# rlvc/FEALESS

Hardware: AMD Instinct MI355X
Metric: frames/sec (640x480 RGB-D x N templates, 20 ICP iters) (higher is better)
Workload: dtype u8

## Files before the change

### fealess_amd/csrc/fl_context.hip

```cpp
#include "fl_internal.h"
#include <stdlib.h>
#include <stdarg.h>
#include <string.h>
#include <algorithm>

int fl_set_error(fl_context *ctx, int code, const char *fmt, ...)
{
  if (ctx) {
    va_list ap;
    va_start(ap, fmt);
    vsnprintf(ctx->err, sizeof(ctx->err), fmt, ap);
    va_end(ap);
  }
  return code;
}

int fl_scratch(fl_context *ctx, size_t bytes, void **out)
{
  if (int rc = fl_context_join(ctx)) return rc;
  if (bytes > ctx->scratch_bytes) {
    if (ctx->scratch) {
      FL_HIP(ctx, hipStreamSynchronize(ctx->stream));
      FL_HIP(ctx, hipFree(ctx->scratch));
      ctx->scratch = nullptr;
// ... 38 lines not shown
  FL_HIP(ctx, hipStreamSynchronize(ctx->stream));
  if (ctx->icp_stream) FL_HIP(ctx, hipStreamSynchronize(ctx->icp_stream));
  ctx->icp_pending = false;
  return FL_OK;
}

int fl_icp_stream(fl_context *ctx, hipStream_t *out)
{
  const long mode = ctx->opt.pipeline_icp;
  if (ctx->icp_stream && ctx->icp_stream_mode != mode) {
    FL_HIP(ctx, hipStreamSynchronize(ctx->icp_stream));
    FL_HIP(ctx, hipStreamDestroy(ctx->icp_stream));
    ctx->icp_stream = nullptr;
  }
  if (!ctx->icp_stream) {
    int least = 0, greatest = 0;
    FL_HIP(ctx, hipDeviceGetStreamPriorityRange(&least, &greatest));
    FL_HIP(ctx, hipStreamCreateWithPriority(&ctx->icp_stream, hipStreamNonBlocking, mode == 2 ? greatest : (mode == 3 ? least : 0)));
    ctx->icp_stream_mode = mode;
  }
  if (!ctx->ev_icp_tail) FL_HIP(ctx, hipEventCreateWithFlags(&ctx->ev_icp_tail, hipEventDisableTiming));
  *out = ctx->icp_stream;
  return FL_OK;
}

extern "C" int fl_abi_version(void) { return FL_ABI_VERSION; }

struct FlOptionName { const char *name, *env; long fl_context::Options::*field; bool hex; long lo, hi; };
static const FlOptionName fl_option_names[] = {
  {"scan_prune", "FL_SCAN_PRUNE", &fl_context::Options::scan_prune, false, 0, 1},
  {"scan_prune_mid", "FL_SCAN_PRUNE_MID", &fl_context::Options::scan_prune_mid, true, -1, 0xFF},
  {"scan_prune_lanes", "FL_SCAN_PRUNE_LANES", &fl_context::Options::scan_prune_lanes, false, 0, 1},
  {"scan_prune_step", "FL_SCAN_PRUNE_STEP", &fl_context::Options::scan_prune_step, false, 0, 8},
  {"icp_wide", "FL_ICP_WIDE", &fl_context::Options::icp_wide, false, -1, 1},
  {"icp_occ", "FL_ICP_OCC", &fl_context::Options::icp_occ, false, 0, 5},
  {"icp_order", "FL_ICP_ORDER", &fl_context::Options::icp_order, false, 0, 1},
  {"icp_wg_per_cu", "FL_ICP_WG_PER_CU", &fl_context::Options::icp_wg_per_cu, false, 0, 3},
  {"eager_frontend", "FL_EAGER_FRONTEND", &fl_context::Options::eager_frontend, false, 0, 1},
  {"dev_poison", "FL_DEV_POISON", &fl_context::Options::dev_poison, false, 0, 1},
  {"ws_pad", "FL_DEV_WS_PAD", &fl_context::Options::ws_pad, false, 0, 16l << 20},
  {"pipeline_icp", "FL_PIPELINE_ICP", &fl_context::Options::pipeline_icp, false, 0, 3},
  {"frontend_chunk_rows", "FL_FRONTEND_CHUNK_ROWS", &fl_context::Options::frontend_chunk_rows, false, 0, 60 * 1024},
  {"scan_run", "FL_SCAN_RUN", &fl_context::Options::scan_run, false, 0, 64},
  {"refine_lds", "FL_REFINE_LDS", &fl_context::Options::refine_lds, false, 0, 2},
  {"refine_lds_bytes", "FL_REFINE_LDS_BYTES", &fl_context::Options::refine_lds_bytes, false, 0, FL_REFINE_LDS_BYTES},
  {"verify_fused", "FL_VERIFY_FUSED", &fl_context::Options::verify_fused, false, 0, 1},
  {"verify_fused_px", "FL_VERIFY_FUSED_PX", &fl_context::Options::verify_fused_px, false, 0, FL_VERIFY_FUSED_PX},
};

static bool fl_option_valid(const FlOptionName &o, long v)
{
  if (v < o.lo || v > o.hi) return false;
  if (o.field == &fl_context::Options::frontend_chunk_rows) return v % 60 == 0;
  if (o.field == &fl_context::Options::verify_fused_px) return v == 0 || v >= FL_WAVE;
  if (o.field == &fl_context::Options::scan_prune_step) return v == 0 || v == 2 || v == 4 || v == 8;
  return o.field != &fl_context::Options::icp_occ || v == 0 || v >= 4;
}

extern "C" int fl_context_create(int device, fl_context **out)
{
  if (!out) return FL_ERR_INVALID;
  *out = nullptr;
  int n = 0;
  if (hipGetDeviceCount(&n) != hipSuccess || n <= 0) return FL_ERR_NO_DEVICE;
  if (device < 0 || device >= n) return FL_ERR_INVALID;
  fl_context *ctx = new fl_context();
  ctx->device = device;
  if (hipSetDevice(device) != hipSuccess ||
      hipStreamCreateWithFlags(&ctx->own_stream, hipStreamNonBlocking) != hipSuccess) {
    delete ctx;
    return FL_ERR_HIP;
  }
  ctx->stream = ctx->own_stream;
  {
    hipDeviceProp_t prop;
    if (hipGetDeviceProperties(&prop, device) == hipSuccess && prop.multiProcessorCount > 0) ctx->cus = prop.multiProcessorCount;
  }
  for (const FlOptionName &o : fl_option_names)
    if (const char *e = getenv(o.env)) {
      const long v = o.hex ? (long)strtoul(e, nullptr, 16) : atol(e);
      if (fl_option_valid(o, v)) ctx->opt.*(o.field) = v;
    }
  *out = ctx;
  return FL_OK;
}

extern "C" void *fl_context_get_stream(fl_context *ctx) { return ctx ? (void *)ctx->stream : nullptr; }
extern "C" int fl_context_get_device(const fl_context *ctx) { return ctx ? ctx->device : -1; }
// ... 525 lines not shown
              ff.qx = (int16_t)((f.x - rx) / Tl);
              ff.qy = (int16_t)((f.y - ry) / Tl);
              ff.label = (uint8_t)f.label;
              ff.pad = 0;
            }
            fine_feat.push_back(ff);
            const FlRect one = {ff.x, ff.y, ff.x, ff.y};
            box = fl_rect_union(box, one);
          }
          fine_hdr.push_back(h);
          fine_box.push_back(FlFineBox{(int16_t)box.x0, (int16_t)box.y0, (int16_t)box.x1, (int16_t)box.y1});
          all = fl_rect_union(all, box);
        }
        if (all.x1 >= all.x0) {
          const FlLevelGeom &gl = det->geom[l];
          const int ww = std::min(all.x1 - all.x0 + 15 * gl.T + 1 + 3, (gl.w + 3) & ~3);
          const int hh = std::min(all.y1 - all.y0 + 15 * gl.T + 1, gl.h);
          const long bytes = (long)fl_refine_pitch(ww, fl_refine_qmask(gl.T)) * hh;
          det->refine_window_max[l] = std::max(det->refine_window_max[l], bytes);
        }
      }
    }
  }
  det->n_pyr = g_idx;
  det->scan_bytes_per_frame = scan_bytes;

  int rc;
  {
    std::vector<FlScanItem> items;
    fl_build_scan_items(scan_hdr, g_idx, M, det->geom[L - 1].WH, det->geom[L - 1].zero_off, scan_off, items);
    det->n_scan_items = (int)items.size();
    det->scan_item_g.clear();
    for (const FlScanItem &it : items) det->scan_item_g.push_back(it.g);
    if ((rc = upload(ctx, items, &det->d_scan_items))) return rc;
  }
  if ((rc = upload(ctx, scan_off, &det->d_scan_off))) return rc;
  if ((rc = upload(ctx, fine_hdr, &det->d_fine_hdr))) return rc;
  if ((rc = upload(ctx, fine_feat, &det->d_fine_feat))) return rc;
  if ((rc = upload(ctx, fine_box, &det->d_fine_box))) return rc;
  if ((rc = upload(ctx, pyr, &det->d_pyr))) return rc;
  if ((rc = upload(ctx, poses, &det->d_poses))) return rc;
  if ((rc = upload(ctx, class_first, &det->d_class_first))) return rc;
  if ((rc = fl_apply_class_filter(det))) return rc;
  {
    const uint16_t **tmp = nullptr;
    if ((rc = upload(ctx, depth_ptrs, (const uint16_t ***)&tmp))) return rc;
    det->d_depth_ptrs = tmp;
  }

  det->w0 = w0;
  det->h0 = h0;
  det->max_batch = max_batch;
  det->eager_env = ctx->opt.eager_frontend != 0;
  det->poison_env = ctx->opt.dev_poison != 0;
  if ((rc = layout_workspace(det, cap))) return rc;
  if ((rc = fl_icp_prepare(det))) return rc;
  FL_HIP(ctx, hipMalloc((void **)&det->d_results, sizeof(fl_recognition_result) * (size_t)max_batch));
  FL_HIP(ctx, hipHostMalloc((void **)&det->h_results, sizeof(fl_recognition_result) * 2 * (size_t)max_batch,
                            hipHostMallocDefault));
  for (auto &e : det->ev) FL_HIP(ctx, hipEventCreate(&e));
  for (int b = 0; b < 2; ++b) {
    FL_HIP(ctx, hipEventCreateWithFlags(&det->ev_done[b], hipEventDisableTiming));
    FL_HIP(ctx, hipEventCreateWithFlags(&det->ev_set_read[b], hipEventDisableTiming));
  }
  det->finalized = true;
  return FL_OK;
// ... 2 lines not shown
```

### fealess_amd/csrc/fl_internal.h

```cpp
#pragma once
#include <hip/hip_runtime.h>
#include <cmath>
#include <stdint.h>
#include <stdio.h>
#include <string>
#include <vector>
#include "../../include/fealess_hip.h"

#define FL_WAVE 64

struct fl_context {
  int device = 0;
  hipStream_t own_stream = nullptr;
  hipStream_t stream = nullptr;
  hipStream_t icp_stream = nullptr;
  long icp_stream_mode = 0;
  hipEvent_t ev_icp_tail = nullptr;
  bool icp_pending = false;
  char err[512] = {0};
  void *scratch = nullptr;
  size_t scratch_bytes = 0;
  void *pinned = nullptr;
  size_t pinned_bytes = 0;
  int cus = 256;
  struct Options {
    long scan_prune = 1;
    long scan_prune_mid = -1;
    long scan_prune_lanes = 1;
    long scan_prune_step = 0;
    long icp_wide = -1;
    long icp_occ = 0;
    long icp_order = 1;
    long icp_wg_per_cu = 0;
    long eager_frontend = 0;
    long dev_poison = 0;
    long ws_pad = 0;
    long pipeline_icp = 3;
    long frontend_chunk_rows = 0;
    long scan_run = 0;
    long refine_lds = 0;
    long refine_lds_bytes = 0;
    long verify_fused = 0;
    long verify_fused_px = 0;
  } opt;
  bool verify_fused_attr = false;
  int detectors = 0;
  bool destroy_pending = false;
};

int fl_set_error(fl_context *ctx, int code, const char *fmt, ...);
int fl_scratch(fl_context *ctx, size_t bytes, void **out);
int fl_pinned(fl_context *ctx, size_t bytes, void **out);
int fl_context_join(fl_context *ctx);
int fl_context_sync_all(fl_context *ctx);
int fl_icp_stream(fl_context *ctx, hipStream_t *out);

#define FL_HIP(ctx, call)                                                                  \
  do {                                                                                     \
    hipError_t e_ = (call);                                                                \
    if (e_ != hipSuccess)                                                                  \
      return fl_set_error((ctx), FL_ERR_HIP, "%s:%d: %s -> %s", __FILE__, __LINE__, #call, \
                          hipGetErrorString(e_));                                          \
// ... 141 lines not shown

struct FlClass {
  std::string id;
  int n_pyramids = 0;
  std::vector<fl_template> templates;
  std::vector<fl_feature> features;
  std::vector<float> poses;
  int first_g = 0;
  uint16_t *d_depths = nullptr;
  std::vector<uint8_t> has_depth;
  int dw = 0, dh = 0;
};

struct FlBatch {
  int n = 0;
  const uint16_t *depth = nullptr;
  size_t depth_stride = 0;
  bool match_only = false;
};

struct fl_detector {
  fl_context *ctx = nullptr;
  int M = 0, L = 0;
  int T[FL_MAX_LEVELS] = {0};
  std::vector<FlClass> classes;
  bool finalized = false;
  int w0 = 0, h0 = 0, max_batch = 0, cap = 0;
  bool cap_hard = false;
  int n_pyr = 0;
  FlLevelGeom geom[FL_MAX_LEVELS];

  FlScanItem *d_scan_items = nullptr;
  int n_scan_items = 0;
  std::vector<int32_t> scan_item_g;
  uint32_t *d_scan_off = nullptr;
  FlFineHdr *d_fine_hdr = nullptr;
  FlFineBox *d_fine_box = nullptr;
  long refine_window_max[FL_MAX_LEVELS] = {0};
  int refine_ran[FL_MAX_LEVELS] = {0};
  FlFineFeat *d_fine_feat = nullptr;
  FlPyrInfo *d_pyr = nullptr;
  int *d_class_first = nullptr;
  uint8_t *d_item_enabled = nullptr;
  std::vector<std::string> class_filter;
  float *d_poses = nullptr;
  const uint16_t **d_depth_ptrs = nullptr;
  int depth_w = 0, depth_h = 0;
  int max_tw = 0, max_th = 0;

  uint8_t *d_ws = nullptr;
  size_t ws_stride = 0;
  size_t off_bgr = 0, off_depth = 0, off_cand = 0, off_count = 0, off_keys = 0, off_match = 0;
  size_t off_icp = 0, off_tmp = 0;
  size_t off_count_set[2] = {0, 0}, off_match_set[2] = {0, 0};
  int set = 0;
  hipEvent_t ev_set_read[2] = {nullptr, nullptr};
  bool set_busy[2] = {false, false};
  size_t off_tiles = 0;
  bool lazy_capable = false;
  bool lazy = false;
  bool eager_env = false, poison_env = false;
  const uint8_t *lazy_bgr = nullptr;
  hipStream_t copy_stream = nullptr;
  uint8_t *d_in[2] = {nullptr, nullptr};
  hipEvent_t ev_up[2] = {nullptr, nullptr}, ev_read[2] = {nullptr, nullptr};
  bool read_pending[2] = {false, false};
// ... 182 lines not shown
```

### fealess_amd/csrc/fl_linemod.hip

```cpp
#include "fl_internal.h"
#include <limits.h>
#include <string.h>
#include <algorithm>
#include <type_traits>

__global__ __launch_bounds__(256) void k_build_lm_generic(FlPlanes pl, int n_mod, int w, int h, int T, int W, int WH, uint32_t stride)
{
  const int p = blockIdx.x * 256 + threadIdx.x;
  const int gi = blockIdx.y;
  const int frame = blockIdx.z / n_mod, m = blockIdx.z - frame * n_mod;
  const uint8_t *q = pl.in + (size_t)frame * pl.in_stride + pl.in_off[m];
  uint8_t *out = pl.out + (size_t)frame * pl.out_stride + pl.out_off[m];
  if (p >= WH) return;
  const int gy = gi / T, gx = gi - gy * T;
  const int yt = p / W, xt = p - yt * W;
  const int y = yt * T + gy, x = xt * T + gx;
  unsigned b = 0;
  const int rmax = min(T, h - y), cmax = min(T, w - x);
  for (int r = 0; r < rmax; ++r) {
    const uint8_t *row = q + (size_t)(y + r) * w + x;
    for (int c = 0; c < cmax; ++c) b |= row[c];
  }
  const unsigned bb = b | (b << 8);
#pragma unroll
// ... 396 lines not shown
  unsigned prune_mid;
  int prune_lanes;
  uint16_t *dbg;
  int dbg_first, dbg_count;
};

typedef unsigned int u32x4 __attribute__((ext_vector_type(4)));
typedef unsigned short u16x2 __attribute__((ext_vector_type(2)));
__device__ __forceinline__ u16x2 pk_bytes_max(uint32_t a)
{
  const uint32_t lo = a & 0x00FF00FFu, hi = (a >> 8) & 0x00FF00FFu;
  return __builtin_elementwise_max(__builtin_bit_cast(u16x2, lo), __builtin_bit_cast(u16x2, hi));
}
__device__ __forceinline__ uint4 ld16(const uint8_t *p)
{
  uint4 v;
  __builtin_memcpy(&v, p, 16);
  return v;
}
#define FL_CONST_AS __attribute__((address_space(4)))
__device__ __forceinline__ uint32_t sload1(const void *p) { return *(const FL_CONST_AS uint32_t *)(uintptr_t)p; }
__device__ __forceinline__ uint32_t rl(uint32_t v, int l) { return (uint32_t)__builtin_amdgcn_readlane((int)v, l); }

#ifndef FL_SCAN_PRUNE_MID
#define FL_SCAN_PRUNE_MID 0x7Fu
#endif
#ifndef FL_SCAN_OFFSETS_AHEAD
#define FL_SCAN_OFFSETS_AHEAD 1
#endif
#ifndef FL_SCAN_WPE
#define FL_SCAN_WPE 5
#endif
#ifndef FL_SCAN_WPE_PRUNED
#define FL_SCAN_WPE_PRUNED 6
#endif
#ifndef FL_SCAN_STEP
#define FL_SCAN_STEP 4
#endif
#ifndef FL_SCAN_TAIL_ALWAYS
#define FL_SCAN_TAIL_ALWAYS 0
#endif
#ifdef FL_SCAN_STATS
#define FL_SCAN_STATS_N (4 + 2 * FL_MAX_FEATURES + 1)
__device__ unsigned long long d_scan_stats[FL_SCAN_STATS_N];
#define FL_SCAN_STAT(i, v) do { if (lane == 0) atomicAdd(&d_scan_stats[i], (unsigned long long)(v)); } while (0)
#else
#define FL_SCAN_STAT(i, v) do { } while (0)
#endif
template <int N> struct ScanInt { static constexpr int value = N; };
template <int WPE, int STEP>
__global__ __launch_bounds__(256) __attribute__((amdgpu_waves_per_eu(WPE, WPE))) void k_scan(ScanArgs a)
{
  static_assert(STEP == 8 || STEP == 4 || STEP == 2, "a group of eight offsets is cut into equal parts");
  const int wave = threadIdx.x >> 6, lane = threadIdx.x & 63;
  const int xcd = blockIdx.x & 7, q = blockIdx.x >> 3;
  const int frame = xcd + 8 * (q / a.bpf);
  if (frame >= a.n_frames) return;
  int it = __builtin_amdgcn_readfirstlane(((q % a.bpf) * 4 + wave) * a.wave_step);
  if (it >= a.n_items) return;
  const int l7 = lane & 7;
  auto request_item = [&](int idx) {
    const uint32_t *p = lane < 16 ? (const uint32_t *)(a.items + idx) + lane : (const uint32_t *)(a.enabled + (idx & ~3));
    return *p;
  };
  uint32_t rec = request_item(it);
  const uint8_t *lm[FL_MAX_MODALITIES];
  for (int m = 0; m < FL_MAX_MODALITIES; ++m) lm[m] = a.ws + (size_t)frame * a.ws_stride + a.lm_off[m];
  const float thr100 = a.threshold / 100.f;
  const unsigned lane_off = (unsigned)lane * 16u;
  const int dbg_first = a.dbg_first;
  const unsigned dbg_count = (unsigned)a.dbg_count;
  const FL_CONST_AS ScanArgs *ka = (const FL_CONST_AS ScanArgs *)__builtin_amdgcn_kernarg_segment_ptr();

  auto scan_item = [&](const uint32_t r) {
    const int g = (int)rl(r, 8), chunk = (int)(rl(r, 9) & 0xFFFFu), nf_all = (int)(rl(r, 9) >> 16);
    const int rP[FL_MAX_MODALITIES] = {(int)rl(r, 10), (int)rl(r, 13)}, rB[FL_MAX_MODALITIES] = {(int)rl(r, 11), (int)rl(r, 14)};
    const uint32_t rN[FL_MAX_MODALITIES] = {rl(r, 12), rl(r, 15)};
    const int j0 = chunk * 1024 + lane * 16;

    uint32_t tot[16];
#pragma unroll
    for (int i = 0; i < 16; ++i) tot[i] = 0;
    const int prune_threshold = (int)(2 * nf_all + thr100 * (2 * nf_all) + 0.5f);
    const bool tapped = (unsigned)(g - dbg_first) < dbg_count;
    const bool prune = a.prune && !tapped;
    const unsigned mid = prune ? a.prune_mid : 0u;
    const bool by_lane = prune && a.prune_lanes;
    uint64_t alive = ~0ull;
    auto still = [&](bool reachable) {
      const uint64_t b = __ballot(reachable) & alive;
      alive = by_lane || b == 0ull ? b : ~0ull;
      return alive != 0ull;
    };
    [[maybe_unused]] int f_done = 0;
    FL_SCAN_STAT(0, 1);
    uint32_t ov = r;
    int o_at = (rN[0] & 0xFFFFu) ? rB[0] : -1;
    int nf = 0;
#pragma unroll
    for (int m = 0; m < FL_MAX_MODALITIES; ++m) {
      if (m >= a.M) break;
      const int P = rP[m], off_begin = rB[m], n_pad = (int)(rN[m] & 0xFFFFu), h_nf = (int)(rN[m] >> 16);
      uint32_t mx_tot = 0;
      if (prune && m > 0) {
#pragma unroll
        for (int i = 0; i < 16; ++i) mx_tot = max(mx_tot, tot[i]);
        if (!still((int)mx_tot + 4 * (nf_all - nf) > prune_threshold)) {
          FL_SCAN_STAT(4 + f_done, 1);
          return;
        }
      }
      nf += h_nf;
      if (chunk * 1024 >= P) continue;
      const uint8_t *lm_u = lm[m] + chunk * 1024;
      const __amdgpu_buffer_rsrc_t rsrc = __builtin_amdgcn_make_buffer_rsrc((void *)(lm_u - 4), 0, 0x7FFFFFFF, 0x00020000);
      uint32_t a0 = 0, a1 = 0, a2 = 0, a3 = 0;
      const unsigned lm_mis = (unsigned)(size_t)lm_u & 3u;
      const int lanes_on = min(64, ((P - chunk * 1024 + 15) >> 4) + 1);
      const uint64_t lanes_mask = lanes_on >= 64 ? ~0ull : (1ull << lanes_on) - 1ull;
      const int next_begin = rB[m + 1 < FL_MAX_MODALITIES ? m + 1 : m];
      for (int k = 0; k < n_pad; k += 8) {
        const int at = off_begin + k;
        if (o_at != at) ov = a.offs[at + l7];
        const int nxt_at = k + 8 < n_pad ? at + 8 : next_begin;
        const uint32_t nxt = a.offs[nxt_at + l7];
        auto add_features = [&](auto s0_, auto n_) {
          constexpr int S0 = decltype(s0_)::value, N = decltype(n_)::value;
          uint32_t o[N];
#pragma unroll
          for (int u = 0; u < N; ++u) o[u] = rl(ov, S0 + u);
          const uint64_t need = (alive | alive << 1) & lanes_mask;
          FL_SCAN_STAT(1, N);
          FL_SCAN_STAT(2, N * __builtin_popcountll(need));
          const bool tail_on = FL_SCAN_TAIL_ALWAYS || (need >> 63) != 0ull;
          uint32_t tail[N];
#pragma unroll
          for (int u = 0; u < N; ++u) tail[u] = 0u;
          if (__builtin_amdgcn_inverse_ballot_w64(need)) {
          uint4 v[N];
          uint32_t e[N];
          unsigned mis_all = 0;
          if (tail_on) {
#pragma unroll
            for (int u = 0; u < N; ++u) tail[u] = sload1(lm_u + o[u] - ((lm_mis + o[u]) & 3u) + 1024);
          }
#pragma unroll
          for (int u = 0; u < N; ++u) {
            const unsigned off = o[u];
            const unsigned mis_u = (lm_mis + off) & 3u;
            mis_all |= mis_u << (4 * u);
            const u32x4 ld = __builtin_amdgcn_raw_buffer_load_b128(rsrc, lane_off, off - mis_u + 4u, 0);
            v[u] = make_uint4(ld.x, ld.y, ld.z, ld.w);
            e[u] = (uint32_t)__builtin_amdgcn_update_dpp((int)tail[u], (int)v[u].x, 0x130, 0xF, 0xF, false);
          }
#pragma unroll
          for (int u = 0; u < N; ++u) {
            const unsigned mis_u = (mis_all >> (4 * u)) & 3u;
            a0 += __builtin_amdgcn_alignbyte(v[u].y, v[u].x, mis_u);
            a1 += __builtin_amdgcn_alignbyte(v[u].z, v[u].y, mis_u);
            a2 += __builtin_amdgcn_alignbyte(v[u].w, v[u].z, mis_u);
            a3 += __builtin_amdgcn_alignbyte(e[u], v[u].w, mis_u);
          }
          if (S0 == 0) asm volatile("" :: "v"(nxt));
          }
          f_done += N;
        };
        auto reachable = [&](int done) {
          const u16x2 b0 = pk_bytes_max(a0), b1 = pk_bytes_max(a1), b2 = pk_bytes_max(a2), b3 = pk_bytes_max(a3);
          const u16x2 bm = __builtin_elementwise_max(__builtin_elementwise_max(b0, b1), __builtin_elementwise_max(b2, b3));
          const int part = (int)max(bm.x, bm.y);
          const int left = nf_all - nf + max(0, h_nf - done);
          if (still((int)mx_tot + part + 4 * left > prune_threshold)) return true;
          FL_SCAN_STAT(4 + f_done, 1);
          return false;
        };
        const bool chk = (mid >> (k >> 3)) & 1u;
        if (STEP == 8 || k == 0) {
          add_features(ScanInt<0>{}, ScanInt<8>{});
          if (chk && !reachable(k + 8)) return;
        } else if (STEP == 4) {
          add_features(ScanInt<0>{}, ScanInt<4>{});
          if (chk && !reachable(k + 4)) return;
          add_features(ScanInt<4>{}, ScanInt<4>{});
          if (chk && !reachable(k + 8)) return;
        } else {
          add_features(ScanInt<0>{}, ScanInt<2>{});
          if (chk && !reachable(k + 2)) return;
          add_features(ScanInt<2>{}, ScanInt<2>{});
          if (chk && !reachable(k + 4)) return;
          add_features(ScanInt<4>{}, ScanInt<2>{});
          if (chk && !reachable(k + 6)) return;
          add_features(ScanInt<6>{}, ScanInt<2>{});
          if (chk && !reachable(k + 8)) return;
        }
        ov = nxt;
        o_at = FL_SCAN_OFFSETS_AHEAD ? nxt_at : -1;
      }
      const uint32_t acc[4] = {a0, a1, a2, a3};
#pragma unroll
      for (int i = 0; i < 16; ++i) {
        uint32_t byte = (acc[i >> 2] >> ((i & 3) * 8)) & 0xFFu;
        tot[i] += (j0 + i < P) ? byte : 0u;
      }
    }
    if (tapped) {
      const FL_CONST_AS ScanArgs *kr = ka;
      asm volatile("" : "+s"(kr));
      const int WH = kr->WH;
      uint16_t *d = kr->dbg + ((size_t)frame * dbg_count + (g - dbg_first)) * WH;
#pragma unroll
      for (int i = 0; i < 16; ++i)
        if (j0 + i < WH) d[j0 + i] = (uint16_t)tot[i];
    }
    const int raw_threshold = (int)(2 * nf + thr100 * (2 * nf) + 0.5f);
    uint32_t mx = 0;
#pragma unroll
    for (int i = 0; i < 16; ++i) mx = max(mx, tot[i]);
    FL_SCAN_STAT(3, 1);
    if ((int)mx <= raw_threshold || !__builtin_amdgcn_inverse_ballot_w64(alive)) return;
    const FL_CONST_AS ScanArgs *kr = ka;
    asm volatile("" : "+s"(kr));
    const int W = kr->W, WH = kr->WH, T = kr->T, cap = kr->cap;
    uint8_t *ws = kr->ws + (size_t)frame * kr->ws_stride;
    int *count = (int *)(ws + kr->off_count);
    FlCand *cand = (FlCand *)(ws + kr->off_cand);
    const int offset = T / 2 + (T % 2 - 1);
#pragma unroll
    for (int i = 0; i < 16; ++i) {
      const int raw = (int)tot[i];
      const int j = j0 + i;
      if (raw > raw_threshold && j < WH) {
        const int rr = j / W, c = j - rr * W;
        const int idx = atomicAdd(count, 1);
        if (idx < cap) {
          FlCand cd;
          cd.x = c * T + offset;
          cd.y = rr * T + offset;
          cd.g = g;
          cd.sim = (raw * 100.f) / (4 * nf) + 0.5f;
          cand[idx] = cd;
        }
      }
    }
  };

  const int it_end = min(a.n_items, it + a.run * a.item_step);
  for (;;) {
    const uint32_t cur = rec;
    const bool cur_on = ((rl(cur, 16) >> ((it & 3) * 8)) & 0xFFu) != 0;
    const int nx = it + a.item_step;
    const bool more = nx < it_end;
    const int nxc = more ? nx : it;
    rec = request_item(nxc);
    if (cur_on) scan_item(cur);
    if (!more) break;
    it = nx;
  }
}

__device__ __noinline__ uint32_t refine_slow_path(const uint8_t *sp, bool in, int xt0, int yt0, int gx, int gy, int T,
                                                  int W, int H, int w)
{
  uint32_t out = 0;
  const int g0 = gy * T + gx, TT = T * T;
  for (int c = 0; c < 4; ++c) {
    int xx = xt0 + c, yy = yt0, gg = g0;
    const int wx = xx >= W ? xx / W : 0;
    xx -= wx * W;
    yy += wx;
    const int wy = yy >= H ? yy / H : 0;
    yy -= wy * H;
// ... 527 lines not shown
    for (int d = 1; d < (int)blockDim.x; d <<= 1) {
      int v = threadIdx.x >= d ? s_scan[threadIdx.x - d] : 0;
      __syncthreads();
      s_scan[threadIdx.x] += v;
      __syncthreads();
    }
    const int pos = s_base + s_scan[threadIdx.x] - flag;
    if (flag) {
      fl_match m;
      m.similarity = __uint_as_float((unsigned)(k.hi >> 32));
      m.template_id = 0x7FFFFFFF - (int)(k.hi & 0xFFFFFFFFu);
      m.class_idx = 0xFFFF - (int)(k.lo >> 32);
      m.y = (0xFFFF - (int)((k.lo >> 16) & 0xFFFF)) - 32768;
      m.x = (0xFFFF - (int)(k.lo & 0xFFFF)) - 32768;
      out[pos] = m;
    }
    __syncthreads();
    if (threadIdx.x == blockDim.x - 1) s_base += s_scan[threadIdx.x];
    __syncthreads();
  }
  if (threadIdx.x == 0) {
    counters[1] = s_base;
    counters[2] = n_raw > a.cap ? 1 : 0;
  }
}

#ifndef FL_SCAN_RUN_AUTO
#define FL_SCAN_RUN_AUTO 8
#endif
#ifndef FL_SCAN_STRIDED
#define FL_SCAN_STRIDED 1
#endif
#define FL_SCAN_FILL 4
static int fl_scan_run(const fl_context *ctx, int items, int n_frames)
{
  if (ctx->opt.scan_run) return (int)ctx->opt.scan_run;
  const long need = (long)FL_SCAN_FILL * ctx->cus * 4 * (ctx->opt.scan_prune ? FL_SCAN_WPE_PRUNED : FL_SCAN_WPE);
  int run = FL_SCAN_RUN_AUTO;
  while (run > 1 && (long)n_frames * ((items + run - 1) / run) < need) run /= 2;
  return run;
}

#ifndef FL_SCAN_STEP_FRAMES
#define FL_SCAN_STEP_FRAMES 256
#endif
static int fl_scan_step(const fl_context *ctx, int n_frames)
{
  if (ctx->opt.scan_prune_step) return (int)ctx->opt.scan_prune_step;
  return n_frames >= FL_SCAN_STEP_FRAMES ? FL_SCAN_STEP : 8;
}

#ifndef FL_REFINE_LDS_FRAMES_PER_CU
#define FL_REFINE_LDS_FRAMES_PER_CU 1
#endif
static bool fl_refine_use_lds(const fl_detector *det, int level, int n_frames, long *budget)
{
  const fl_context *ctx = det->ctx;
  *budget = ctx->opt.refine_lds_bytes ? ctx->opt.refine_lds_bytes : (long)FL_REFINE_LDS_BYTES;
  if (ctx->opt.refine_lds == 1 || det->refine_window_max[level] > *budget) return false;
  return ctx->opt.refine_lds == 2 || n_frames >= FL_REFINE_LDS_FRAMES_PER_CU * ctx->cus;
}

extern "C" int fl_dev_refine_pitch(int width, int T) { return fl_refine_pitch(width, fl_refine_qmask(T)); }
extern "C" int fl_dev_refine_plan(const int32_t *rects, int n, int max_len, long budget, int T, int32_t *uni)
{
  FlRect u;
  const int len = fl_refine_plan(rects, n, max_len, budget, fl_refine_qmask(T), &u);
  if (uni) { uni[0] = u.x0; uni[1] = u.y0; uni[2] = u.x1; uni[3] = u.y1; }
  return len;
}
extern "C" int fl_dev_refine_kernel(const fl_detector *det, int level)
{
  return det && level >= 0 && level < det->L - 1 ? det->refine_ran[level] : -1;
}
extern "C" long fl_dev_refine_window_max(const fl_detector *det, int level)
{
  return det && level >= 0 && level < det->L - 1 ? det->refine_window_max[level] : -1;
}

static int launch_scan_refine_sort(fl_detector *det, int n_frames, float threshold, uint16_t *dbg, int dbg_first,
                                   int dbg_count)
{
// ... 7 lines not shown
    a.ws = det->d_ws;
    a.ws_stride = det->ws_stride;
    for (int m = 0; m < FL_MAX_MODALITIES; ++m) a.lm_off[m] = g.lm_off[m < M ? m : 0];
    a.off_count = det->off_count;
    a.off_cand = det->off_cand;
    a.M = M;
    a.W = g.W;
    a.WH = g.WH;
    a.T = g.T;
    a.cap = det->cap;
    a.threshold = threshold;
    a.prune = ctx->opt.scan_prune != 0;
    a.prune_mid = ctx->opt.scan_prune_mid >= 0 ? (unsigned)ctx->opt.scan_prune_mid : FL_SCAN_PRUNE_MID;
    a.prune_lanes = ctx->opt.scan_prune_lanes != 0;
    a.dbg = dbg;
    a.dbg_first = dbg_first;
    a.dbg_count = dbg ? dbg_count : 0;
    a.items = det->d_scan_items;
    a.n_items = det->n_scan_items;
    const int items = det->n_scan_items;
    if (items > 0) {
      a.run = fl_scan_run(ctx, items, n_frames);
      const int waves = (items + a.run - 1) / a.run;
      a.bpf = (waves + 3) / 4;
#if FL_SCAN_STRIDED
      a.wave_step = 1;
      a.item_step = a.bpf * 4;
#else
      a.wave_step = a.run;
      a.item_step = 1;
#endif
      a.n_frames = n_frames;
      dim3 grid((unsigned)(a.bpf * ((n_frames + 7) / 8) * 8));
      if (!a.prune) hipLaunchKernelGGL((k_scan<FL_SCAN_WPE, 8>), grid, dim3(256), 0, ctx->stream, a);
      else switch (fl_scan_step(ctx, n_frames)) {
      case 2: hipLaunchKernelGGL((k_scan<FL_SCAN_WPE_PRUNED, 2>), grid, dim3(256), 0, ctx->stream, a); break;
      case 4: hipLaunchKernelGGL((k_scan<FL_SCAN_WPE_PRUNED, 4>), grid, dim3(256), 0, ctx->stream, a); break;
      default: hipLaunchKernelGGL((k_scan<FL_SCAN_WPE_PRUNED, 8>), grid, dim3(256), 0, ctx->stream, a); break;
      }
      FL_HIP(ctx, hipGetLastError());
#ifdef FL_SCAN_STATS
      {
        unsigned long long st[FL_SCAN_STATS_N], zero[FL_SCAN_STATS_N] = {0};
        FL_HIP(ctx, hipStreamSynchronize(ctx->stream));
        FL_HIP(ctx, hipMemcpyFromSymbol(st, HIP_SYMBOL(d_scan_stats), sizeof(st)));
        FL_HIP(ctx, hipMemcpyToSymbol(HIP_SYMBOL(d_scan_stats), zero, sizeof(zero)));
        fprintf(stderr, "k_scan: %d frames, %llu items, %.2f feature loads and %.1f lane-loads per item, %llu items to their end; ended "
                "after f features:", n_frames, st[0], st[0] ? (double)st[1] / st[0] : 0.0, st[0] ? (double)st[2] / st[0] : 0.0, st[3]);
        for (int f = 0; f + 4 < FL_SCAN_STATS_N; ++f)
          if (st[4 + f]) fprintf(stderr, " %d: %llu", f, st[4 + f]);
        fprintf(stderr, "\n");
      }
#endif
    }
  }
  if (det->have_times) FL_HIP(ctx, hipEventRecord(det->ev[3], ctx->stream));
  for (int l = L - 2; l >= 0; --l) {
    const FlLevelGeom &g = det->geom[l];
    RefineArgs a;
    const bool lazy_level = det->lazy;
    a.hdr = det->d_fine_hdr;
    a.feat = det->d_fine_feat;
    a.ws = det->d_ws;
    a.ws_stride = det->ws_stride;
    for (int m = 0; m < FL_MAX_MODALITIES; ++m) a.spread_off[m] = g.spread_off[m < M ? m : 0];
    a.off_count = det->off_count;
    a.off_cand = det->off_cand;
    a.M = M;
    a.Lm1 = L - 1;
    a.level = l;
    a.w = g.w;
    a.h = g.h;
    a.T = g.T;
    a.W = g.W;
    a.H = g.H;
    a.cap = det->cap;
    a.threshold = threshold;
    if (lazy_level) {
      if (det->have_times) FL_HIP(ctx, hipEventRecord(det->ev[8 + 2 * l], ctx->stream));
      hipLaunchKernelGGL(k_mark_tiles, dim3(n_frames), dim3(256), 0, ctx->stream, a, det->off_tiles);
      FL_HIP(ctx, hipGetLastError());
      int rc = fl_launch_lazy_level(det, n_frames, l);
// ... 785 lines not shown
```

Before: 89290.

## Restructure scan kernel with larger first piece, packed totals and fewer VGPRs

The scan kernel now accumulates a first piece of 12 (configurable) features before its first prune check, chosen at launch from the median feature count and threshold. Per-pixel totals are packed as 16-bit pairs to cut registers. Loads are issued with a bounded in-flight window, the tail byte is loaded by buffer load, and flags are kept in scalar registers. The waves-per-EU target for the pruned kernel rises from 6 to 8. This aims at higher occupancy and less per-feature overhead, at the cost of checking prune later and more template instantiations.

```diff
diff --git a/fealess_amd/csrc/fl_context.hip b/fealess_amd/csrc/fl_context.hip
--- a/fealess_amd/csrc/fl_context.hip
+++ b/fealess_amd/csrc/fl_context.hip
@@ -94,6 +94,7 @@
   {"scan_prune_mid", "FL_SCAN_PRUNE_MID", &fl_context::Options::scan_prune_mid, true, -1, 0xFF},
   {"scan_prune_lanes", "FL_SCAN_PRUNE_LANES", &fl_context::Options::scan_prune_lanes, false, 0, 1},
   {"scan_prune_step", "FL_SCAN_PRUNE_STEP", &fl_context::Options::scan_prune_step, false, 0, 8},
+  {"scan_first", "FL_SCAN_FIRST", &fl_context::Options::scan_first, false, 0, 16},
   {"icp_wide", "FL_ICP_WIDE", &fl_context::Options::icp_wide, false, -1, 1},
   {"icp_occ", "FL_ICP_OCC", &fl_context::Options::icp_occ, false, 0, 5},
   {"icp_order", "FL_ICP_ORDER", &fl_context::Options::icp_order, false, 0, 1},
@@ -116,6 +117,7 @@
   if (o.field == &fl_context::Options::frontend_chunk_rows) return v % 60 == 0;
   if (o.field == &fl_context::Options::verify_fused_px) return v == 0 || v >= FL_WAVE;
   if (o.field == &fl_context::Options::scan_prune_step) return v == 0 || v == 2 || v == 4 || v == 8;
+  if (o.field == &fl_context::Options::scan_first) return v == 0 || v == 8 || v == 12 || v == 14 || v == 16;
   return o.field != &fl_context::Options::icp_occ || v == 0 || v >= 4;
 }
 
@@ -707,6 +709,10 @@
     det->n_scan_items = (int)items.size();
     det->scan_item_g.clear();
     for (const FlScanItem &it : items) det->scan_item_g.push_back(it.g);
+    std::vector<int> nfs;
+    for (const FlScanItem &it : items) nfs.push_back((int)(it.chunk_nf >> 16));
+    if (!nfs.empty()) std::nth_element(nfs.begin(), nfs.begin() + nfs.size() / 2, nfs.end());
+    det->scan_nf_typical = nfs.empty() ? 0 : nfs[nfs.size() / 2];
     if ((rc = upload(ctx, items, &det->d_scan_items))) return rc;
   }
   if ((rc = upload(ctx, scan_off, &det->d_scan_off))) return rc;
diff --git a/fealess_amd/csrc/fl_internal.h b/fealess_amd/csrc/fl_internal.h
--- a/fealess_amd/csrc/fl_internal.h
+++ b/fealess_amd/csrc/fl_internal.h
@@ -28,6 +28,7 @@
     long scan_prune_mid = -1;
     long scan_prune_lanes = 1;
     long scan_prune_step = 0;
+    long scan_first = 0;
     long icp_wide = -1;
     long icp_occ = 0;
     long icp_order = 1;
@@ -235,6 +236,7 @@
 
   FlScanItem *d_scan_items = nullptr;
   int n_scan_items = 0;
+  int scan_nf_typical = 0;
   std::vector<int32_t> scan_item_g;
   uint32_t *d_scan_off = nullptr;
   FlFineHdr *d_fine_hdr = nullptr;
diff --git a/fealess_amd/csrc/fl_linemod.hip b/fealess_amd/csrc/fl_linemod.hip
--- a/fealess_amd/csrc/fl_linemod.hip
+++ b/fealess_amd/csrc/fl_linemod.hip
@@ -452,7 +452,7 @@
 #define FL_SCAN_WPE 5
 #endif
 #ifndef FL_SCAN_WPE_PRUNED
-#define FL_SCAN_WPE_PRUNED 6
+#define FL_SCAN_WPE_PRUNED 8
 #endif
 #ifndef FL_SCAN_STEP
 #define FL_SCAN_STEP 4
@@ -461,17 +461,18 @@
 #define FL_SCAN_TAIL_ALWAYS 0
 #endif
 #ifdef FL_SCAN_STATS
-#define FL_SCAN_STATS_N (4 + 2 * FL_MAX_FEATURES + 1)
+#define FL_SCAN_STATS_N (4 + 2 * FL_MAX_FEATURES + 1 + 1)
 __device__ unsigned long long d_scan_stats[FL_SCAN_STATS_N];
 #define FL_SCAN_STAT(i, v) do { if (lane == 0) atomicAdd(&d_scan_stats[i], (unsigned long long)(v)); } while (0)
 #else
 #define FL_SCAN_STAT(i, v) do { } while (0)
 #endif
 template <int N> struct ScanInt { static constexpr int value = N; };
-template <int WPE, int STEP>
+template <int WPE, int STEP, int FIRST>
 __global__ __launch_bounds__(256) __attribute__((amdgpu_waves_per_eu(WPE, WPE))) void k_scan(ScanArgs a)
 {
   static_assert(STEP == 8 || STEP == 4 || STEP == 2, "a group of eight offsets is cut into equal parts");
+  static_assert(FIRST == 8 || FIRST == 12 || FIRST == 14 || FIRST == 16, "the first piece ends inside the second group, at an even feature");
   const int wave = threadIdx.x >> 6, lane = threadIdx.x & 63;
   const int xcd = blockIdx.x & 7, q = blockIdx.x >> 3;
   const int frame = xcd + 8 * (q / a.bpf);
@@ -479,52 +480,77 @@
   int it = __builtin_amdgcn_readfirstlane(((q % a.bpf) * 4 + wave) * a.wave_step);
   if (it >= a.n_items) return;
   const int l7 = lane & 7;
+  const FL_CONST_AS ScanArgs *ka = (const FL_CONST_AS ScanArgs *)__builtin_amdgcn_kernarg_segment_ptr();
+  auto kargs = [&]() {
+    const FL_CONST_AS ScanArgs *kr = ka;
+    asm volatile("" : "+s"(kr));
+    return kr;
+  };
   auto request_item = [&](int idx) {
     const uint32_t *p = lane < 16 ? (const uint32_t *)(a.items + idx) + lane : (const uint32_t *)(a.enabled + (idx & ~3));
     return *p;
   };
+  enum : unsigned { F_PRUNE = 0x100u, F_BY_LANE = 0x200u, F_TAPPED = 0x400u, F_TAPS = 0x800u, F_M2 = 0x1000u };
+  const unsigned kflags = (a.prune ? F_PRUNE | (a.prune_mid & 0xFFu) | (a.prune_lanes ? F_BY_LANE : 0u) : 0u) | (a.dbg_count ? F_TAPS : 0u) |
+                          (a.M > 1 ? F_M2 : 0u);
   uint32_t rec = request_item(it);
   const uint8_t *lm[FL_MAX_MODALITIES];
   for (int m = 0; m < FL_MAX_MODALITIES; ++m) lm[m] = a.ws + (size_t)frame * a.ws_stride + a.lm_off[m];
   const float thr100 = a.threshold / 100.f;
   const unsigned lane_off = (unsigned)lane * 16u;
-  const int dbg_first = a.dbg_first;
-  const unsigned dbg_count = (unsigned)a.dbg_count;
-  const FL_CONST_AS ScanArgs *ka = (const FL_CONST_AS ScanArgs *)__builtin_amdgcn_kernarg_segment_ptr();
 
   auto scan_item = [&](const uint32_t r) {
+    auto field = [&](int i) {
+      uint32_t rr = r;
+      asm volatile("" : "+v"(rr));
+      return rl(rr, i);
+    };
     const int g = (int)rl(r, 8), chunk = (int)(rl(r, 9) & 0xFFFFu), nf_all = (int)(rl(r, 9) >> 16);
-    const int rP[FL_MAX_MODALITIES] = {(int)rl(r, 10), (int)rl(r, 13)}, rB[FL_MAX_MODALITIES] = {(int)rl(r, 11), (int)rl(r, 14)};
-    const uint32_t rN[FL_MAX_MODALITIES] = {rl(r, 12), rl(r, 15)};
     const int j0 = chunk * 1024 + lane * 16;
 
-    uint32_t tot[16];
-#pragma unroll
-    for (int i = 0; i < 16; ++i) tot[i] = 0;
+    uint32_t tp[8];
+#pragma unroll
+    for (int i = 0; i < 8; ++i) tp[i] = 0;
+    auto tot_at = [&](int i) { return (tp[2 * (i >> 2) + (i & 1)] >> (((i >> 1) & 1) * 16)) & 0xFFFFu; };
+    auto tot_max = [&]() {
+      u16x2 m = __builtin_bit_cast(u16x2, tp[0]);
+#pragma unroll
+      for (int i = 1; i < 8; ++i) m = __builtin_elementwise_max(m, __builtin_bit_cast(u16x2, tp[i]));
+      return (uint32_t)max(m.x, m.y);
+    };
     const int prune_threshold = (int)(2 * nf_all + thr100 * (2 * nf_all) + 0.5f);
-    const bool tapped = (unsigned)(g - dbg_first) < dbg_count;
-    const bool prune = a.prune && !tapped;
-    const unsigned mid = prune ? a.prune_mid : 0u;
-    const bool by_lane = prune && a.prune_lanes;
+    unsigned flags_ = kflags;
+    const unsigned flags_m2 = kflags & F_M2;
+    if (kflags & F_TAPS) {
+      const FL_CONST_AS ScanArgs *ki = kargs();
+      if ((unsigned)(g - ki->dbg_first) < (unsigned)ki->dbg_count) flags_ = F_TAPPED | flags_m2;
+    }
+    const unsigned flags = flags_;
+    auto flag = [&](unsigned bits) {
+      unsigned f = flags;
+      asm volatile("" : "+s"(f));
+      return (f & bits) != 0u;
+    };
     uint64_t alive = ~0ull;
     auto still = [&](bool reachable) {
       const uint64_t b = __ballot(reachable) & alive;
-      alive = by_lane || b == 0ull ? b : ~0ull;
+      alive = flag(F_BY_LANE) || b == 0ull ? b : ~0ull;
       return alive != 0ull;
     };
     [[maybe_unused]] int f_done = 0;
     FL_SCAN_STAT(0, 1);
     uint32_t ov = r;
-    int o_at = (rN[0] & 0xFFFFu) ? rB[0] : -1;
+    int o_at = (rl(r, 12) & 0xFFFFu) ? (int)rl(r, 11) : -1;
     int nf = 0;
 #pragma unroll
     for (int m = 0; m < FL_MAX_MODALITIES; ++m) {
-      if (m >= a.M) break;
-      const int P = rP[m], off_begin = rB[m], n_pad = (int)(rN[m] & 0xFFFFu), h_nf = (int)(rN[m] >> 16);
+      if (m > 0 && !flag(F_M2)) break;
+      const uint32_t rN = m == 0 ? rl(r, 12) : field(12 + 3 * m);
+      const int P = (int)(m == 0 ? rl(r, 10) : field(10 + 3 * m)), off_begin = (int)(m == 0 ? rl(r, 11) : field(11 + 3 * m));
+      const int n_pad = (int)(rN & 0xFFFFu), h_nf = (int)(rN >> 16);
       uint32_t mx_tot = 0;
-      if (prune && m > 0) {
-#pragma unroll
-        for (int i = 0; i < 16; ++i) mx_tot = max(mx_tot, tot[i]);
+      if (m > 0 && flag(F_PRUNE)) {
+        mx_tot = tot_max();
         if (!still((int)mx_tot + 4 * (nf_all - nf) > prune_threshold)) {
           FL_SCAN_STAT(4 + f_done, 1);
           return;
@@ -538,108 +564,158 @@
       const unsigned lm_mis = (unsigned)(size_t)lm_u & 3u;
       const int lanes_on = min(64, ((P - chunk * 1024 + 15) >> 4) + 1);
       const uint64_t lanes_mask = lanes_on >= 64 ? ~0ull : (1ull << lanes_on) - 1ull;
-      const int next_begin = rB[m + 1 < FL_MAX_MODALITIES ? m + 1 : m];
-      for (int k = 0; k < n_pad; k += 8) {
-        const int at = off_begin + k;
-        if (o_at != at) ov = a.offs[at + l7];
-        const int nxt_at = k + 8 < n_pad ? at + 8 : next_begin;
-        const uint32_t nxt = a.offs[nxt_at + l7];
-        auto add_features = [&](auto s0_, auto n_) {
+      auto next_begin = [&]() { return m + 1 < FL_MAX_MODALITIES ? (int)field(11 + 3 * (m + 1)) : off_begin; };
+      uint32_t nxt = 0;
+      auto request = [&](int at) { return a.offs[at + l7]; };
+      {
+        auto piece = [&](auto s0_, auto n_, auto tail_, const uint32_t ov2, const uint32_t tv) {
+          constexpr int S0 = decltype(s0_)::value, N = decltype(n_)::value, InFlight = N < 8 ? N : 8;
+          constexpr bool TAIL = decltype(tail_)::value != 0;
+          uint4 v[InFlight];
+          unsigned mis_all = 0;
+          auto issue = [&](const int u) {
+            unsigned off = rl(S0 + u < 8 ? ov : ov2, (S0 + u) & 7);
+            if (u >= InFlight) asm("" : "+s"(off) : "v"(a0), "v"(a1), "v"(a2), "v"(a3));
+            const unsigned mis_u = (lm_mis + off) & 3u;
+            mis_all |= mis_u << (2 * u);
+            const u32x4 ld = __builtin_amdgcn_raw_buffer_load_b128(rsrc, lane_off, off - mis_u + 4u, 0);
+            v[u % InFlight] = make_uint4(ld.x, ld.y, ld.z, ld.w);
+          };
+          auto take = [&](const int u) {
+            const unsigned mis_u = (mis_all >> (2 * u)) & 3u;
+            const uint4 x = v[u % InFlight];
+            uint32_t e = (uint32_t)__builtin_amdgcn_update_dpp(0, (int)x.x, 0x130, 0xF, 0xF, true);
+            if (TAIL) {
+              const uint32_t t = rl(tv, S0 + u);
+              e = lane == 63 ? t : e;
+            }
+            a0 += __builtin_amdgcn_alignbyte(x.y, x.x, mis_u);
+            a1 += __builtin_amdgcn_alignbyte(x.z, x.y, mis_u);
+            a2 += __builtin_amdgcn_alignbyte(x.w, x.z, mis_u);
+            a3 += __builtin_amdgcn_alignbyte(e, x.w, mis_u);
+          };
+#pragma unroll
+          for (int u = 0; u < InFlight; ++u) issue(u);
+#pragma unroll
+          for (int u = 0; u < N; ++u) {
+            take(u);
+            if (u + InFlight < N) issue(u + InFlight);
+          }
+        };
+        auto add_features = [&](auto s0_, auto n_, const uint32_t ov2) {
           constexpr int S0 = decltype(s0_)::value, N = decltype(n_)::value;
-          uint32_t o[N];
-#pragma unroll
-          for (int u = 0; u < N; ++u) o[u] = rl(ov, S0 + u);
           const uint64_t need = (alive | alive << 1) & lanes_mask;
           FL_SCAN_STAT(1, N);
           FL_SCAN_STAT(2, N * __builtin_popcountll(need));
           const bool tail_on = FL_SCAN_TAIL_ALWAYS || (need >> 63) != 0ull;
-          uint32_t tail[N];
-#pragma unroll
-          for (int u = 0; u < N; ++u) tail[u] = 0u;
+          uint32_t tv = 0;
+          if (tail_on && (unsigned)(lane - S0) < (unsigned)N) {
+            const uint32_t of = lane < 8 ? ov : ov2;
+            tv = __builtin_amdgcn_raw_buffer_load_b32(rsrc, of - ((lm_mis + of) & 3u) + 4u + 1024u, 0, 0);
+          }
           if (__builtin_amdgcn_inverse_ballot_w64(need)) {
-          uint4 v[N];
-          uint32_t e[N];
-          unsigned mis_all = 0;
-          if (tail_on) {
-#pragma unroll
-            for (int u = 0; u < N; ++u) tail[u] = sload1(lm_u + o[u] - ((lm_mis + o[u]) & 3u) + 1024);
-          }
-#pragma unroll
-          for (int u = 0; u < N; ++u) {
-            const unsigned off = o[u];
-            const unsigned mis_u = (lm_mis + off) & 3u;
-            mis_all |= mis_u << (4 * u);
-            const u32x4 ld = __builtin_amdgcn_raw_buffer_load_b128(rsrc, lane_off, off - mis_u + 4u, 0);
-            v[u] = make_uint4(ld.x, ld.y, ld.z, ld.w);
-            e[u] = (uint32_t)__builtin_amdgcn_update_dpp((int)tail[u], (int)v[u].x, 0x130, 0xF, 0xF, false);
-          }
-#pragma unroll
-          for (int u = 0; u < N; ++u) {
-            const unsigned mis_u = (mis_all >> (4 * u)) & 3u;
-            a0 += __builtin_amdgcn_alignbyte(v[u].y, v[u].x, mis_u);
-            a1 += __builtin_amdgcn_alignbyte(v[u].z, v[u].y, mis_u);
-            a2 += __builtin_amdgcn_alignbyte(v[u].w, v[u].z, mis_u);
-            a3 += __builtin_amdgcn_alignbyte(e[u], v[u].w, mis_u);
-          }
-          if (S0 == 0) asm volatile("" :: "v"(nxt));
+            if (tail_on) piece(s0_, n_, ScanInt<1>{}, ov2, tv);
+            else piece(s0_, n_, ScanInt<0>{}, ov2, tv);
+            if (S0 == 0) asm volatile("" :: "v"(nxt));
           }
           f_done += N;
         };
-        auto reachable = [&](int done) {
+        auto reachable = [&](int done, [[maybe_unused]] bool first_piece) {
           const u16x2 b0 = pk_bytes_max(a0), b1 = pk_bytes_max(a1), b2 = pk_bytes_max(a2), b3 = pk_bytes_max(a3);
           const u16x2 bm = __builtin_elementwise_max(__builtin_elementwise_max(b0, b1), __builtin_elementwise_max(b2, b3));
           const int part = (int)max(bm.x, bm.y);
           const int left = nf_all - nf + max(0, h_nf - done);
           if (still((int)mx_tot + part + 4 * left > prune_threshold)) return true;
           FL_SCAN_STAT(4 + f_done, 1);
+          if (first_piece) FL_SCAN_STAT(FL_SCAN_STATS_N - 1, 1);
           return false;
         };
-        const bool chk = (mid >> (k >> 3)) & 1u;
-        if (STEP == 8 || k == 0) {
-          add_features(ScanInt<0>{}, ScanInt<8>{});
-          if (chk && !reachable(k + 8)) return;
-        } else if (STEP == 4) {
-          add_features(ScanInt<0>{}, ScanInt<4>{});
-          if (chk && !reachable(k + 4)) return;
-          add_features(ScanInt<4>{}, ScanInt<4>{});
-          if (chk && !reachable(k + 8)) return;
-        } else {
-          add_features(ScanInt<0>{}, ScanInt<2>{});
-          if (chk && !reachable(k + 2)) return;
-          add_features(ScanInt<2>{}, ScanInt<2>{});
-          if (chk && !reachable(k + 4)) return;
-          add_features(ScanInt<4>{}, ScanInt<2>{});
-          if (chk && !reachable(k + 6)) return;
-          add_features(ScanInt<6>{}, ScanInt<2>{});
-          if (chk && !reachable(k + 8)) return;
+        int k = 0;
+        if (n_pad > 0) {
+          if (o_at != off_begin) ov = request(off_begin);
+          const int nxt_at = 8 < n_pad ? off_begin + 8 : next_begin();
+          nxt = request(nxt_at);
+          if (FIRST > 8 && n_pad > 8) {
+            const int nx2_at = 16 < n_pad ? off_begin + 16 : next_begin();
+            const uint32_t nx2 = request(nx2_at);
+            add_features(ScanInt<0>{}, ScanInt<FIRST>{}, nxt);
+            asm volatile("" :: "v"(nx2));
+            if (flag(2u) && !reachable(FIRST, true)) return;
+            ov = nxt;
+            if (FIRST == 12 && STEP == 2) {
+              add_features(ScanInt<4>{}, ScanInt<2>{}, 0u);
+              if (flag(2u) && !reachable(14, false)) return;
+            } else if (FIRST == 12) {
+              add_features(ScanInt<4>{}, ScanInt<4>{}, 0u);
+              if (flag(2u) && !reachable(16, false)) return;
+            }
+            if (FIRST == 14 || (FIRST == 12 && STEP == 2)) {
+              add_features(ScanInt<6>{}, ScanInt<2>{}, 0u);
+              if (flag(2u) && !reachable(16, false)) return;
+            }
+            ov = nx2;
+            o_at = FL_SCAN_OFFSETS_AHEAD ? nx2_at : -1;
+            k = 16;
+          } else {
+            add_features(ScanInt<0>{}, ScanInt<8>{}, 0u);
+            if (flag(1u) && !reachable(8, true)) return;
+            ov = nxt;
+            o_at = FL_SCAN_OFFSETS_AHEAD ? nxt_at : -1;
+            k = 8;
+          }
         }
-        ov = nxt;
-        o_at = FL_SCAN_OFFSETS_AHEAD ? nxt_at : -1;
+        for (; k < n_pad; k += 8) {
+          const int at = off_begin + k;
+          if (o_at != at) ov = request(at);
+          const int nxt_at = k + 8 < n_pad ? at + 8 : next_begin();
+          nxt = request(nxt_at);
+          const bool chk = flag(1u << (k >> 3));
+          if (STEP == 8) {
+            add_features(ScanInt<0>{}, ScanInt<8>{}, 0u);
+            if (chk && !reachable(k + 8, false)) return;
+          } else if (STEP == 4) {
+            add_features(ScanInt<0>{}, ScanInt<4>{}, 0u);
+            if (chk && !reachable(k + 4, false)) return;
+            add_features(ScanInt<4>{}, ScanInt<4>{}, 0u);
+            if (chk && !reachable(k + 8, false)) return;
+          } else {
+            add_features(ScanInt<0>{}, ScanInt<2>{}, 0u);
+            if (chk && !reachable(k + 2, false)) return;
+            add_features(ScanInt<2>{}, ScanInt<2>{}, 0u);
+            if (chk && !reachable(k + 4, false)) return;
+            add_features(ScanInt<4>{}, ScanInt<2>{}, 0u);
+            if (chk && !reachable(k + 6, false)) return;
+            add_features(ScanInt<6>{}, ScanInt<2>{}, 0u);
+            if (chk && !reachable(k + 8, false)) return;
+          }
+          ov = nxt;
+          o_at = FL_SCAN_OFFSETS_AHEAD ? nxt_at : -1;
+        }
       }
       const uint32_t acc[4] = {a0, a1, a2, a3};
-#pragma unroll
-      for (int i = 0; i < 16; ++i) {
-        uint32_t byte = (acc[i >> 2] >> ((i & 3) * 8)) & 0xFFu;
-        tot[i] += (j0 + i < P) ? byte : 0u;
-      }
-    }
-    if (tapped) {
-      const FL_CONST_AS ScanArgs *kr = ka;
-      asm volatile("" : "+s"(kr));
+      const int nv = P - j0;
+#pragma unroll
+      for (int q = 0; q < 4; ++q) {
+        const int c = nv - 4 * q;
+        const uint32_t w = acc[q] & (c >= 4 ? ~0u : c <= 0 ? 0u : (1u << (8 * c)) - 1u);
+        tp[2 * q] += w & 0x00FF00FFu;
+        tp[2 * q + 1] += (w >> 8) & 0x00FF00FFu;
+      }
+    }
+    const int g_end = (int)field(8);
+    if (flag(F_TAPPED)) {
+      const FL_CONST_AS ScanArgs *kr = kargs();
       const int WH = kr->WH;
-      uint16_t *d = kr->dbg + ((size_t)frame * dbg_count + (g - dbg_first)) * WH;
+      uint16_t *d = kr->dbg + ((size_t)frame * (unsigned)kr->dbg_count + (g_end - kr->dbg_first)) * WH;
 #pragma unroll
       for (int i = 0; i < 16; ++i)
-        if (j0 + i < WH) d[j0 + i] = (uint16_t)tot[i];
+        if (j0 + i < WH) d[j0 + i] = (uint16_t)tot_at(i);
     }
     const int raw_threshold = (int)(2 * nf + thr100 * (2 * nf) + 0.5f);
-    uint32_t mx = 0;
-#pragma unroll
-    for (int i = 0; i < 16; ++i) mx = max(mx, tot[i]);
+    const uint32_t mx = tot_max();
     FL_SCAN_STAT(3, 1);
     if ((int)mx <= raw_threshold || !__builtin_amdgcn_inverse_ballot_w64(alive)) return;
-    const FL_CONST_AS ScanArgs *kr = ka;
-    asm volatile("" : "+s"(kr));
+    const FL_CONST_AS ScanArgs *kr = kargs();
     const int W = kr->W, WH = kr->WH, T = kr->T, cap = kr->cap;
     uint8_t *ws = kr->ws + (size_t)frame * kr->ws_stride;
     int *count = (int *)(ws + kr->off_count);
@@ -647,7 +723,7 @@
     const int offset = T / 2 + (T % 2 - 1);
 #pragma unroll
     for (int i = 0; i < 16; ++i) {
-      const int raw = (int)tot[i];
+      const int raw = (int)tot_at(i);
       const int j = j0 + i;
       if (raw > raw_threshold && j < WH) {
         const int rr = j / W, c = j - rr * W;
@@ -656,7 +732,7 @@
           FlCand cd;
           cd.x = c * T + offset;
           cd.y = rr * T + offset;
-          cd.g = g;
+          cd.g = g_end;
           cd.sim = (raw * 100.f) / (4 * nf) + 0.5f;
           cand[idx] = cd;
         }
@@ -1250,10 +1326,11 @@
 #define FL_SCAN_STRIDED 1
 #endif
 #define FL_SCAN_FILL 4
+#define FL_SCAN_FILL_WAVES 6
 static int fl_scan_run(const fl_context *ctx, int items, int n_frames)
 {
   if (ctx->opt.scan_run) return (int)ctx->opt.scan_run;
-  const long need = (long)FL_SCAN_FILL * ctx->cus * 4 * (ctx->opt.scan_prune ? FL_SCAN_WPE_PRUNED : FL_SCAN_WPE);
+  const long need = (long)FL_SCAN_FILL * ctx->cus * 4 * (ctx->opt.scan_prune ? FL_SCAN_FILL_WAVES : FL_SCAN_WPE);
   int run = FL_SCAN_RUN_AUTO;
   while (run > 1 && (long)n_frames * ((items + run - 1) / run) < need) run /= 2;
   return run;
@@ -1266,6 +1343,18 @@
 {
   if (ctx->opt.scan_prune_step) return (int)ctx->opt.scan_prune_step;
   return n_frames >= FL_SCAN_STEP_FRAMES ? FL_SCAN_STEP : 8;
+}
+
+#ifndef FL_SCAN_FIRST
+#define FL_SCAN_FIRST 12
+#endif
+static int fl_scan_first(const fl_detector *det, int n_frames, float threshold)
+{
+  const fl_context *ctx = det->ctx;
+  if (ctx->opt.scan_first) return (int)ctx->opt.scan_first;
+  const int nf = det->scan_nf_typical;
+  const int raw_threshold = (int)(2 * nf + threshold / 100.f * (2 * nf) + 0.5f);
+  return n_frames >= FL_SCAN_STEP_FRAMES && 4 * nf - raw_threshold > 28 ? FL_SCAN_FIRST : 8;
 }
 
 #ifndef FL_REFINE_LDS_FRAMES_PER_CU
@@ -1339,12 +1428,23 @@
 #endif
       a.n_frames = n_frames;
       dim3 grid((unsigned)(a.bpf * ((n_frames + 7) / 8) * 8));
-      if (!a.prune) hipLaunchKernelGGL((k_scan<FL_SCAN_WPE, 8>), grid, dim3(256), 0, ctx->stream, a);
+#define FL_SCAN_LAUNCH(WPE, STEP, FIRST) hipLaunchKernelGGL((k_scan<WPE, STEP, FIRST>), grid, dim3(256), 0, ctx->stream, a)
+#define FL_SCAN_LAUNCH_STEP(STEP) \
+      switch (first) { \
+      case 12: FL_SCAN_LAUNCH(FL_SCAN_WPE_PRUNED, STEP, 12); break; \
+      case 14: FL_SCAN_LAUNCH(FL_SCAN_WPE_PRUNED, STEP, 14); break; \
+      case 16: FL_SCAN_LAUNCH(FL_SCAN_WPE_PRUNED, STEP, 16); break; \
+      default: FL_SCAN_LAUNCH(FL_SCAN_WPE_PRUNED, STEP, 8); break; \
+      }
+      const int first = fl_scan_first(det, n_frames, threshold);
+      if (!a.prune) FL_SCAN_LAUNCH(FL_SCAN_WPE, 8, 8);
       else switch (fl_scan_step(ctx, n_frames)) {
-      case 2: hipLaunchKernelGGL((k_scan<FL_SCAN_WPE_PRUNED, 2>), grid, dim3(256), 0, ctx->stream, a); break;
-      case 4: hipLaunchKernelGGL((k_scan<FL_SCAN_WPE_PRUNED, 4>), grid, dim3(256), 0, ctx->stream, a); break;
-      default: hipLaunchKernelGGL((k_scan<FL_SCAN_WPE_PRUNED, 8>), grid, dim3(256), 0, ctx->stream, a); break;
-      }
+      case 2: FL_SCAN_LAUNCH_STEP(2); break;
+      case 4: FL_SCAN_LAUNCH_STEP(4); break;
+      default: FL_SCAN_LAUNCH_STEP(8); break;
+      }
+#undef FL_SCAN_LAUNCH_STEP
+#undef FL_SCAN_LAUNCH
       FL_HIP(ctx, hipGetLastError());
 #ifdef FL_SCAN_STATS
       {
@@ -1353,8 +1453,9 @@
         FL_HIP(ctx, hipMemcpyFromSymbol(st, HIP_SYMBOL(d_scan_stats), sizeof(st)));
         FL_HIP(ctx, hipMemcpyToSymbol(HIP_SYMBOL(d_scan_stats), zero, sizeof(zero)));
         fprintf(stderr, "k_scan: %d frames, %llu items, %.2f feature loads and %.1f lane-loads per item, %llu items to their end; ended "
-                "after f features:", n_frames, st[0], st[0] ? (double)st[1] / st[0] : 0.0, st[0] ? (double)st[2] / st[0] : 0.0, st[3]);
-        for (int f = 0; f + 4 < FL_SCAN_STATS_N; ++f)
+                "by a first piece's check %llu; after f features:", n_frames, st[0], st[0] ? (double)st[1] / st[0] : 0.0,
+                st[0] ? (double)st[2] / st[0] : 0.0, st[3], st[FL_SCAN_STATS_N - 1]);
+        for (int f = 0; f + 5 < FL_SCAN_STATS_N; ++f)
           if (st[4 + f]) fprintf(stderr, " %d: %llu", f, st[4 + f]);
         fprintf(stderr, "\n");
       }
```

Result: faster. 90430, median of 6 (+1.3%).
